# suryatmodulus/livekit-server

Hardware: AMD Instinct MI355X
Metric: forwarded RTP pkts/sec per GPU & node (bit-exact) + % HBM roofline (higher is better)
Workload: dtype u8; 1 GPU; configs[1]: 100 rooms x 10 participants per GPU, VP8 3-layer simulcast + Opus, 18000 DownTracks, 2% loss, 1% reorder, layer switching; batch=1 s of media per step, step=raw datagrams -> Buffer.calc -> forward (lkf_ingest_device + lkf_run), parallelism=room-sharded x1

## Files before the change

### livekit-server_amd/csrc/engine.cpp

```cpp
#include <hip/hip_runtime.h>

#include <algorithm>
#include <chrono>
#include <cmath>
#include <cstdio>
#include <cstdlib>
#include <cstring>
#include <atomic>
#include <map>
#include <mutex>
#include <string>
#include <tuple>
#include <vector>

#include "../../include/lkfwd.h"
#include "ctl_csr.h"
#include "dev_buf.h"
#include "fwd_state.h"
#include "hip_own.h"
#include "kernels.h"

using namespace lkf;

namespace {

struct DevRegistry {
  std::mutex m;
  std::map<uintptr_t, size_t> a;
};
DevRegistry &dreg() {
  static DevRegistry r;
  return r;
}

}

int lkf::dev_alloc(void **p, size_t bytes) {
  *p = nullptr;
  const hipError_t r = hipMalloc(p, bytes);
  if (r == hipSuccess) {
    std::lock_guard<std::mutex> g(dreg().m);
    dreg().a[reinterpret_cast<uintptr_t>(*p)] = bytes;
  }
  return int(r);
}

int lkf::dev_free(void *p) {
  {
    std::lock_guard<std::mutex> g(dreg().m);
    dreg().a.erase(reinterpret_cast<uintptr_t>(p));
  }
  return int(hipFree(p));
}

namespace {

bool dev_range_ok(const void *src, size_t n) {
  const uintptr_t s = reinterpret_cast<uintptr_t>(src);
  std::lock_guard<std::mutex> g(dreg().m);
  auto it = dreg().a.upper_bound(s);
  if (it == dreg().a.begin()) return false;
  --it;
  return s >= it->first && n <= it->second && s - it->first <= it->second - n;
}

constexpr int kStatsWords = 4 + LKF_DROP_NREASONS;
constexpr uint32_t kIdle = 0xffffffffu;

struct Knobs {
  int cuSplit = 0;
// ... 29 lines not shown
    k.debugDD = num("LKF_DEBUG_DD", 0) != 0;
    k.skipBktStore = num("LKF_SKIP_BKT_STORE", 0) != 0;
    k.nackAlone = num("LKF_NACK_ALONE", 0) != 0;
    return k;
  }
};

template <typename Keep>
hipError_t cu_mask_stream(Stream &s, int dev, Keep keep) {
  int ncu = 256;
  (void)hipDeviceGetAttribute(&ncu, hipDeviceAttributeMultiprocessorCount, dev);
  std::vector<uint32_t> m(size_t((ncu + 31) / 32), 0);
  for (int i = 0; i < ncu; i++)
    if (keep(i % 32)) m[size_t(i / 32)] |= 1u << (i % 32);
  return hipExtStreamCreateWithCUMask(s.put(), uint32_t(m.size()), m.data());
}

struct BatchCtx {
  DevBuf<uint32_t> dTBegin, dTEnd, dTRuns, dErr;
  DevBuf<uint64_t> dSlotBase, dPartA, dTot;
  DevBuf<FwdRec> dRecs;
  DevBuf<FwdBase> dFBase;
  DevBuf<FwdBase> dWide;
  DevBuf<uint32_t> dFwdCnt;
  DevBuf<uint64_t> dFwdBytes, dRecBase, dByteBase;
  DevBuf<uint32_t> dGFirst;
  DevBuf<uint32_t> dTwccBase;
  DevBuf<uint32_t> dLayerList, dLayerBefore, dLayerCnt;
  DevBuf<lkf_out> dOut;
  DevBuf<uint8_t> dOutArena;
  int egress = LKF_EGRESS_WIRE;
  DevBuf<lkf_pre> dPre;
  DevBuf<uint32_t> dPreGSum;
  DevBuf<uint64_t> dPreGBase, dPreTot;
  DevBuf<uint64_t> dStats;
  DevBuf<lkf_pkt> dPktsOwn;
  DevBuf<uint8_t> dArenaOwn;
  DevBuf<lkf_raw_pkt> dRawPkts;
  DevBuf<uint64_t> dBktStore;
  DevBuf<lkf_pkt_dd> dDDIn;
  DevBuf<DDPkt> dDDPkt;
  DevBuf<uint8_t> dDDArena;
  DevBuf<uint64_t> dDDUsed;
  DevBuf<uint16_t> dDDSpill;
  DevBuf<DevEvent> dEvents;
  DevBuf<uint32_t> dEvOff;
  DevBuf<uint32_t> dEvLane;
  Event prepped;
  Event pulled;
  Event decided;
  Event sent;
  Event emitted;
  Event ingested;
  bool fromIngest = false;
  bool prepByIngest = false;
  uint32_t prepNT = 0, prepND = 0;
  DevBuf<uint64_t> dITotal;
  bool used = false;
  bool keyed = false;
  DevBuf<uint8_t> dProt;
  bool protectedRun = false;
  DevBuf<RunDesc> dDesc;
  StagePair stage;
  uint32_t stageCap = 0;
  StageGraph gPrep[2], gScan, gCtl;
  void forget_pull_graphs() { gPrep[0].epoch = gPrep[1].epoch = gCtl.epoch = 0; }
};

}

struct lkf_engine {
  int dev = 0;
  Knobs knobs;
  double hp[9] = {};
  CtlCsr csr;
  Stream own;
  Stream d2hS;
  Stream prepS;
  Stream ingS;
  Stream decS;
  Stream emitS;
  Stream sendS;
  Stream sideS;
  std::vector<int32_t> dtTransport;
  DevBuf<uint32_t> dTwccCtrD, dTwccCtrT, dTwccTOff, dTwccTList;
  uint32_t nTwccT = 0;
  bool anyTwcc = false, twccDirty = false;
  Event sideFork, sideDone[2];
  bool sidePending[2] = {false, false};
  Event bktDone[2];
  bool bktPending[2] = {false, false};
  hipStream_t cur = nullptr;
  Event inEv;
  Event bktEv;
  bool bktStorePending = false;
  lkf_cfg cfg{};
  int egress = LKF_EGRESS_WIRE;
  std::string err;

  std::vector<lkf_track_params> tracks;
  std::vector<uint32_t> trackDD;
  std::vector<uint8_t> trackActive;
  std::vector<lkf_downtrack_params> dtp;
  std::vector<uint8_t> active;
  std::vector<uint8_t> seqRM;
  bool schedDirty = true;
// ... 78 lines not shown
  const uint64_t *curNDev = nullptr;
  bool ingestStarted = false;

#ifndef LKF_CTX
#define LKF_CTX 3
#endif
  static constexpr int kCtx = LKF_CTX;
  BatchCtx ctx[kCtx];
  uint64_t nRuns = 0;
  int lastCtx = -1;
  PinnedBuf bounce;

  DevBuf<lkf_nack> dNacks;
  DevBuf<uint32_t> dNackG, dNackValid;
  DevBuf<lkf_rtx> dRtx;
  DevBuf<lkf_raw_pkt> dRtxSrc;
  DevBuf<uint32_t> dRtxLen;
  DevBuf<uint64_t> dRtxOff;
  DevBuf<uint8_t> dRtxIn, dRtxOut;

  DevBuf<TrackerState> dTrk;
  uint32_t nTrk = 0;
  DevBuf<int32_t> dTrkIds;
  DevBuf<lkf_tracker_status> dTrkOut;
  DevBuf<RedEncState> dRedEnc;
  DevBuf<RedDecState> dRedDec;
  struct RedScratch {
    DevBuf<lkf_pkt> in, out;
    DevBuf<uint8_t> inArena, outArena;
    DevBuf<uint32_t> g, cnt;
    DevBuf<int32_t> map;
    DevBuf<uint64_t> off;
  } red;
  DevBuf<lkf_allocation> dLastAlloc;
  DevBuf<lkf_alloc_req> dAllocReq;
  DevBuf<int64_t> dAllocCapacity;
  DevBuf<lkf_allocation> dAllocOut;
  DevBuf<uint8_t> dSrm;
  uint64_t srmStride = 0;
  uint32_t srmCap = 0;
  DevBuf<lkf_pad_req> dPadReq;
  DevBuf<uint64_t> dPadOff;
  DevBuf<uint32_t> dPadCnt;
  DevBuf<lkf_out> dPadOut;
  DevBuf<uint8_t> dPadArena;

  DevBuf<uint16_t> dSns;
  DevBuf<lkf_seq_meta> dSeqOut;
  DevBuf<uint32_t> dSeqN;

  static constexpr int kRing = 256;
  Event ring[kRing][5];
  uint32_t emitGrid = 2048;
  std::vector<lkf_transport_params> transports;
  DevBuf<lkf_transport_params> dTransports;
  DevBuf<SrtpKeys> dSrtpKeys;
  DevBuf<uint32_t> dAesTab;
  DevBuf<SrtpDT> dSrtpDT;
  Event protRing[256][2];
  std::vector<uint8_t> protRun;
  DevBuf<SrtpRx> dSrtpRx, dSrtpRxSpec;
  DevBuf<uint32_t> dRxRange, dRxAuth;
  DevBuf<SrtpRxSpec> dRxSpec;
  DevBuf<lkf_srtp_rx_result> dRxRes;
  DevBuf<uint8_t> dSrtpStage;
  DevBuf<lkf_raw_pkt> dSrtpPktsIn;
  Event rxRing[256][2];
  uint64_t nUnprotects = 0;
  uint32_t lastUnprotectN = 0;
  uint32_t maxStreams = 0;
  DevBuf<DevStream> dStreams;
  DevBuf<StreamHot> dStreamHot;
  DevBuf<uint64_t> dHist;
  DevBuf<uint32_t> dRxGap;
  DevBuf<RangeEntry> dStreamRings;
  DevBuf<uint32_t> dTwcc;
  DevBuf<BucketState> dBkt;
  DevBuf<uint32_t> dBktTag;
  DevBuf<uint64_t> dBktOwner;
  uint32_t bktEpoch = 0;
  DevBuf<uint8_t> dBktRing;
  uint64_t bktSlots = 0;
  DevBuf<int32_t> dBktStream;
  DevBuf<uint16_t> dBktSn;
  DevBuf<uint64_t> dPos, dIPartA, dITotal;
  DevBuf<uint32_t> dITRuns, dIErr;
  struct IngSet {
    DevBuf<IngParsed> parsed;
    DevBuf<lkf_flow> flows;
    DevBuf<uint32_t> fwd, tBegin, tEnd, list, listCnt;
    DevBuf<uint32_t> nackInfo, nackPairOff, nackPairCnt;
    DevBuf<lkf_nack_pair> nackPairs;
    DevBuf<NackIn> nackIn;
  } ing[2];
  int ingPar = 0;
  DevBuf<NackState> dNack;
  uint32_t nackPairCap = 0;
  DevBuf<uint64_t> dNackRecPos, dNackPairPos, dNackTot;
  DevBuf<uint64_t> dNackPartA;
  DevBuf<lkf_rtcp_nack> dNackOut;
  DevBuf<lkf_nack_pair> dNackPairsOut;
  uint32_t lastIngestN = 0;
  const lkf_raw_pkt *ingRaws = nullptr;
  uint32_t nRooms = 0;
  DevBuf<uint32_t> dRoomPartOff, dPartId, dPartMicOff, dMics, dRoomId;
  DevBuf<lkf_speaker> dSpkSlots;
// ... 414 lines not shown
  A(e->dSSGap.alloc(size_t(c.max_downtracks) * kGapWords));
  A(e->dSSRing.alloc(size_t(c.max_downtracks) * kSnInfoSize));
  A(e->dDTs.alloc(c.max_downtracks));
  A(e->dRm.alloc(size_t(c.max_downtracks) * kRangeCap));
  A(e->dVc.alloc(c.max_downtracks));
  A(e->dSeq.alloc(size_t(c.max_downtracks) * c.seq_size));
  e->srmCap = seqrm_cap(c.seq_size);
  e->srmStride = seqrm_stride(e->srmCap);
  A(e->dSrm.alloc(size_t(c.max_downtracks) * e->srmStride));
  A(e->dLastAlloc.alloc(c.max_downtracks));
  A(e->dCum.alloc(kStatsWords));
  A(e->dSticky.alloc(4));
  A(e->dPerm.alloc(c.max_downtracks));
  A(e->dDTOffs.alloc(size_t(c.max_downtracks) * kDTOffsWords));
  const size_t nparts = scan_state_words(c.max_downtracks);
  for (auto &x : e->ctx) {
    A(x.dTBegin.alloc(c.max_tracks));
    A(x.dTEnd.alloc(c.max_tracks));
    A(x.dTRuns.alloc(c.max_tracks));
    A(x.dErr.alloc(4));
    A(x.dSlotBase.alloc(c.max_downtracks));
    A(x.dPartA.alloc(nparts));
    A(hipMemset(x.dPartA, 0, nparts * sizeof(uint64_t)));
    A(x.dTot.alloc(4));
    A(x.dRecs.alloc(c.max_batch_tuples));
    A(x.dFBase.alloc(c.max_downtracks));
    A(x.dWide.alloc(c.max_batch_tuples));
    A(x.dFwdCnt.alloc(c.max_downtracks));
    A(x.dFwdBytes.alloc(c.max_downtracks));
    A(x.dRecBase.alloc(c.max_downtracks));
    A(x.dByteBase.alloc(c.max_downtracks));
    A(x.dGFirst.alloc(c.max_out_pkts / 64 + 2));
    A(x.dTwccBase.alloc(c.max_downtracks));
    A(x.dLayerList.alloc(3 * size_t(c.max_batch_pkts) + 64));
    A(x.dLayerBefore.alloc(3 * size_t(c.max_batch_pkts) + 64));
    A(x.dLayerCnt.alloc(3 * size_t(c.max_tracks)));
    A(x.dOut.alloc(c.max_out_pkts));
    A(x.dOutArena.alloc(c.max_out_bytes + 64));
    A(x.dStats.alloc(size_t(kStatsWords) * (1 + kStatCopies)));
    A(x.dPktsOwn.alloc(c.max_batch_pkts));
    A(x.dArenaOwn.alloc(c.max_batch_arena + 64));
    A(x.dRawPkts.alloc(c.max_batch_pkts));
    A(x.dBktStore.alloc(c.max_batch_pkts));
    A(x.dDesc.alloc(1));
    A(x.dEvents.alloc(4096));
    A(x.dEvLane.alloc(4096));
    A(x.decided.create(false));
    A(x.prepped.create(false));
    A(x.pulled.create(false));
    A(x.emitted.create(false));
    A(x.ingested.create(false));
    A(x.dITotal.alloc(2));
    A(x.sent.create(false));
  }
  for (auto &r : e->ring)
    for (auto &ev : r) A(ev.create(true));
  A(e->scanRead.create(false));
  e->maxStreams = c.max_streams ? c.max_streams : 3 * c.max_tracks;
  A(e->dStreams.alloc(e->maxStreams));
  A(e->dStreamHot.alloc(e->maxStreams));
  A(e->dHist.alloc(size_t(e->maxStreams) * kHistWords));
  A(e->dRxGap.alloc(size_t(e->maxStreams) * kGapWords));
  A(e->dStreamRings.alloc(size_t(e->maxStreams) * kRangeCap));
  for (auto &g : e->ing) {
    A(g.parsed.alloc(c.max_batch_pkts));
    A(g.flows.alloc(c.max_batch_pkts));
    A(g.fwd.alloc(c.max_batch_pkts));
    A(g.tBegin.alloc(c.max_tracks));
    A(g.tEnd.alloc(c.max_tracks));
    A(g.list.alloc(3 * size_t(c.max_batch_pkts) + 64));
    A(g.listCnt.alloc(3 * size_t(c.max_tracks)));
  }
  A(e->dTwcc.alloc(c.max_batch_pkts));
  A(e->dPos.alloc(c.max_batch_pkts));
  const size_t ipart = scan_state_words(c.max_batch_pkts);
  A(e->dIPartA.alloc(ipart));
  A(hipMemset(e->dIPartA, 0, ipart * sizeof(uint64_t)));
  A(e->dITotal.alloc(2));
  A(e->dITRuns.alloc(c.max_tracks));
  A(e->dIErr.alloc(4));
  if (ok) {
    A(hipMemset(e->dSeq, 0, size_t(c.max_downtracks) * c.seq_size * sizeof(SeqMeta)));
    A(hipMemset(e->dRm, 0, size_t(c.max_downtracks) * kRangeCap * sizeof(RangeEntry)));
    A(hipMemset(e->dVc, 0, size_t(c.max_downtracks) * sizeof(VP8Cold)));
    A(hipMemset(e->dSrm, 0, size_t(c.max_downtracks) * e->srmStride));
    A(hipMemset(e->dHot, 0, size_t(c.max_downtracks) * sizeof(DTHot)));
    A(hipMemset(e->dDTs, 0, size_t(c.max_downtracks) * sizeof(DevDT)));
    A(hipMemset(e->dDTCum, 0, size_t(c.max_downtracks) * sizeof(DTCum)));
    A(hipMemset(e->dSeqDDIdx, 0xff, size_t(c.max_downtracks) * sizeof(uint32_t)));
    A(hipMemset(e->dTracks, 0, size_t(c.max_tracks) * sizeof(DevTrack)));
    A(hipMemset(e->dStreamHot, 0, size_t(e->maxStreams) * sizeof(StreamHot)));
    A(hipMemset(e->dStreamRings, 0, size_t(e->maxStreams) * kRangeCap * sizeof(RangeEntry)));
    A(hipMemset(e->dHist, 0, size_t(e->maxStreams) * kHistWords * sizeof(uint64_t)));
    {
      lkf_allocation d = {};
      d.pause_reason = 3;
      d.target_spatial = d.target_temporal = d.request_spatial = d.max_spatial = d.max_temporal = -1;
      std::vector<lkf_allocation> v(c.max_downtracks, d);
      A(hipMemcpy(e->dLastAlloc, v.data(), v.size() * sizeof(lkf_allocation), hipMemcpyHostToDevice));
    }
    A(hipMemset(e->dCum, 0, kStatsWords * sizeof(uint64_t)));
    A(hipMemset(e->dSticky, 0, 4 * sizeof(uint32_t)));
    for (auto &x : e->ctx) {
      A(hipMemset(x.dArenaOwn, 0, c.max_batch_arena + 64));
      A(hipMemset(x.dTot, 0, 4 * sizeof(uint64_t)));
      A(hipMemset(x.dStats, 0, size_t(kStatsWords) * (1 + kStatCopies) * sizeof(uint64_t)));
      A(hipMemset(x.dErr, 0, 4 * sizeof(uint32_t)));
    }
    A(hipDeviceSynchronize());
  }
  if (!ok) {
    lkf_destroy(e);
    return nullptr;
  }
  int cus = 256;
  (void)hipDeviceGetAttribute(&cus, hipDeviceAttributeMultiprocessorCount, hip_device);
  e->emitGrid = uint32_t(cus) * uint32_t(kn.emitWgPerCU);
  return e;
}

void lkf_destroy(lkf_engine *e) {
  if (!e) return;
  if (e->knobs.hostProf && e->hp[5] > 0)
    fprintf(stderr,
            "lkf host ms/run: pre %.4f stage-wait %.4f csr %.4f copies %.4f launches %.4f total %.4f (%d runs)\n",
            e->hp[0] / e->hp[5], e->hp[1] / e->hp[5], e->hp[2] / e->hp[5], e->hp[6] / e->hp[5],
            e->hp[3] / e->hp[5], e->hp[4] / e->hp[5], int(e->hp[5]));
  if (e->knobs.hostProf && e->hp[8] > 0)
    fprintf(stderr, "lkf host ms/ingest: %.4f (%d ingests: the launches of the Buffer.calc chain, no host wait)\n",
            e->hp[7] / e->hp[8], int(e->hp[8]));
  (void)hipSetDevice(e->dev);
  if (e->cur && e->cur != e->own) (void)hipStreamSynchronize(e->cur);
  if (e->own) (void)hipStreamSynchronize(e->own);
  if (e->ingS) (void)hipStreamSynchronize(e->ingS);
  if (e->prepS) (void)hipStreamSynchronize(e->prepS);
  if (e->decS) (void)hipStreamSynchronize(e->decS);
  if (e->emitS) (void)hipStreamSynchronize(e->emitS);
  if (e->sendS) (void)hipStreamSynchronize(e->sendS);
  if (e->sideS) (void)hipStreamSynchronize(e->sideS);
  if (e->d2hS) (void)hipStreamSynchronize(e->d2hS);
  (void)hipDeviceSynchronize();
  delete e;
}

int32_t lkf_add_track(lkf_engine *e, const lkf_track_params *p) {
  if (!e || !p) return LKF_EINVAL;
  if (e->tracks.size() >= e->cfg.max_tracks) return LKF_ENOSPC;
  int32_t h = int32_t(e->tracks.size());
  e->tracks.push_back(*p);
  uint32_t ddIdx = 0xffffffffu;
  if (track_has_dd(*p)) ddIdx = e->nDDTracks++;
  e->trackDD.push_back(ddIdx);
  e->trackActive.push_back(1);
  e->trkSR.emplace_back();
  std::memcpy(e->trkSR.back().offs, p->layer_offsets, 9 * sizeof(uint32_t));
  e->pendTracks.push_back(to_dev_track(*p, ddIdx));
  e->schedDirty = true;
  return h;
}

static bool at_key_valid(int32_t kind, int64_t key) {
  if (kind == LKF_AT_PKT) return key >= 0 && key <= int64_t(0xffffffffu);
  if (kind == LKF_AT_DATAGRAM) return key >= 0;
  return kind == LKF_AT_ARRIVAL_NS;
}

int lkf_set_layer_offsets_key(lkf_engine *e, int32_t track, const uint32_t offsets[9], int32_t kind, int64_t key) {
  if (!e || !offsets || track < 0 || track >= int32_t(e->tracks.size())) return LKF_EINVAL;
  if (!at_key_valid(kind, key)) return LKF_EINVAL;
  lkf_engine::TrackOp op;
  op.track = uint32_t(track);
  op.at = kind == LKF_AT_PKT ? uint32_t(key) : 0u;
  op.kind = kind;
  op.key = key;
  std::memcpy(op.offs, offsets, sizeof(op.offs));
  std::memcpy(e->trkSR[size_t(track)].offs, offsets, sizeof(op.offs));
  e->trkOps.push_back(op);
  if (kind != LKF_AT_PKT) e->keyedPending = true;
  return LKF_OK;
}
// ... 726 lines not shown
    q.list = e->dSeqDDList;
    q.n = e->nSeqDD;
    q.hot = e->dHot;
    q.seq = e->dSeq;
    q.seqSize = e->cfg.seq_size;
    q.srm = e->dSrm;
    q.srmStride = e->srmStride;
    q.srmCap = e->srmCap;
    q.ddIdx = e->dSeqDDIdx;
    q.seqDD = e->dSeqDD;
    q.recs = x.dRecs;
    q.fbase = x.dFBase;
    q.wide = x.dWide;
    q.slotBase = x.dSlotBase;
    q.fwdCnt = x.dFwdCnt;
    q.pkts = e->curPkts;
    q.ddArena = x.dDDArena;
    HIPCHK(launch_seq_dd(s, q), "sequencer dd");
  }
  return LKF_OK;
}

static EmitArgs emit_args(const lkf_engine *e, const BatchCtx &x, const RunCtx &r) {
  EmitArgs m{};
  m.perm = e->dPerm;
  m.recBase = x.dRecBase;
  m.byteBase = x.dByteBase;
  m.gFirst = x.dGFirst;
  m.slotBase = x.dSlotBase;
  m.totals = x.dTot + 2;
  m.recs = x.dRecs;
  m.fbase = x.dFBase;
  m.wide = x.dWide;
  m.pkts = e->curPkts;
  m.arena = e->curArena;
  m.dts = e->dDTs;
  m.ndts = r.nd;
  m.out = x.dOut;
  m.outArena = x.dOutArena;
  m.outCap = e->cfg.max_out_pkts;
  m.outByteCap = e->cfg.max_out_bytes;
  m.err = x.dErr;
  m.ddArena = e->ddAlloc ? x.dDDArena.get() : nullptr;
  m.maxDts = e->cfg.max_downtracks;
  m.npkts = e->curN;
  m.tupleCap = e->cfg.max_batch_tuples;
  m.arenaLen = e->curArenaLen;
  m.ddCap = x.dDDArena.cap();
  m.twccBase = e->anyTwcc ? x.dTwccBase.get() : nullptr;
  m.gCap = e->cfg.max_out_pkts / 64 + 2;
  return m;
}

static uint32_t emit_grid(const lkf_engine *e) {
  return e->knobs.emitPersistent ? e->emitGrid : uint32_t(((e->cfg.max_out_pkts + 63) / 64 + 7) / 8 * 8);
}

static uint32_t emit_lds_pad(const lkf_engine *e, const RunCtx &r) {
  const bool lowFanout = uint64_t(r.nd) < uint64_t(e->knobs.emitCapFanout) * std::max<uint32_t>(1, r.nt);
  return r.ingestFed && lowFanout ? e->knobs.emitLdsPad : 0;
}

static int enqueue_emit(lkf_engine *e, BatchCtx &x, const RunCtx &r) {
  hipStream_t es = e->emitS;
  HIPCHK(hipStreamWaitEvent(es, x.decided, 0), "wait decided");
  HIPCHK(hipEventRecord(r.rg[3], es), "event");
  const EmitArgs m = emit_args(e, x, r);
  const uint32_t grid = emit_grid(e);
  x.egress = e->egress;
  if (x.egress == LKF_EGRESS_PREFIX) {
    EmitPrefixLaunch q;
    q.pre = x.dPre;
    q.gSum = x.dPreGSum;
    q.gBase = x.dPreGBase;
    q.total = x.dPreTot;
    if (r.nd)
      HIPCHK(launch_emit_prefix(es, m, grid, q), "emit prefix");
    else
      HIPCHK(hipMemsetAsync(x.dPreTot, 0, sizeof(uint64_t), es), "emit prefix");
  } else if (r.nd) {
    HIPCHK(launch_emit(es, m, grid, emit_lds_pad(e, r)), "emit");
  }
  HIPCHK(hipEventRecord(r.rg[4], es), "event");
  HIPCHK(launch_accumulate(es, x.dStats, x.dTot, e->dCum, x.dErr, e->dSticky), "accumulate");
  if (e->bktStorePending) {
    HIPCHK(hipEventRecord(x.sent, e->sendS), "event");
    HIPCHK(hipStreamWaitEvent(es, x.sent, 0), "wait bucket store");
  }
  e->bktStorePending = false;
  HIPCHK(hipEventRecord(x.emitted, es), "event");
  return LKF_OK;
}

static void finish_run(lkf_engine *e, BatchCtx &x, const RunCtx &r) {
  if (e->knobs.hostProf && e->nRuns >= 3) {
    e->hp[0] += ms_between(r.tp0, r.tp1);
    e->hp[1] += ms_between(r.tp1, r.tp2);
    e->hp[2] += ms_between(r.tp2, r.tp25);
    e->hp[6] += ms_between(r.tp25, r.tp3);
    e->hp[3] += ms_since(r.tp3);
    e->hp[4] += ms_since(r.tp0);
    e->hp[5] += 1;
  }
  x.used = true;
  x.protectedRun = false;
  if (!e->protRun.empty()) e->protRun[e->nRuns % 256] = 0;
  e->lastCtx = r.ci;
  e->nRuns++;
  e->haveBatch = false;
  e->curNDev = nullptr;
  e->curDD = nullptr;
}

int lkf_run(lkf_engine *e, void *stream) {
  if (!e) return LKF_EINVAL;
  HIPCHK(hipSetDevice(e->dev), "hipSetDevice");
  if (int rc = flush_topology(e)) return rc;
  if (e->schedDirty) {
    if (int rc = rebuild_sched(e)) return rc;
  }
  if (e->twccDirty) {
    if (int rc = rebuild_twcc(e)) return rc;
  }
  RunCtx r{};
  r.ci = int(e->nRuns % lkf_engine::kCtx);
  BatchCtx &x = e->ctx[r.ci];
  if (!e->haveBatch) {
    e->curPkts = x.dPktsOwn;
    e->curArena = x.dArenaOwn;
    e->curOwned = e->curDDOwned = true;
    e->curN = 0;
    e->curNDev = nullptr;
    e->curArenaLen = 0;
    e->curFromIngest = false;
  }
  r.tp0 = clk::now();
  hipStream_t us = stream ? reinterpret_cast<hipStream_t>(stream) : e->own;
  e->cur = us;
  r.nt = uint32_t(e->tracks.size());
  r.nd = uint32_t(e->dtp.size());
  r.nl = uint32_t(e->sched.size());
  r.rg = e->ring[e->nRuns % lkf_engine::kRing];
  expand_track_ops(e, r);
  r.keyed = e->keyedPending;
  e->keyedPending = false;
  if (r.keyed) {
    if (int rc = refuse_mixed_kinds(e, r)) return rc;
  }
  for (const auto &op : e->trkOps)
    std::memcpy(e->tracks[op.track].layer_offsets, op.offs, sizeof(op.offs));
  e->trkOps.clear();
  if (int rc = wait_inputs(e, x, r, us)) return rc;
  if (int rc = stage_ctl(e, x, r)) return rc;
  if (int rc = enqueue_prep(e, x, r)) return rc;
  if (int rc = enqueue_decide(e, x, r)) return rc;
// ... 2636 lines not shown
```

### livekit-server_amd/csrc/forward_kernels.hip

```cpp
#include <hip/hip_runtime.h>

#include "../../include/lkfwd.h"
#ifndef LKF_SVC_STATS
#define LKF_SVC_STATS 0
#endif
#if LKF_SVC_STATS
__device__ unsigned long long g_svc[64 * 48];
#define SVC_ADD(k, v) atomicAdd(&g_svc[(blockIdx.x & 63) * 48 + (k)], (unsigned long long)(v))
#endif
#include "dd_device.h"
#include "fwd_state.h"
#include "kernels.h"
#include "sender_device.h"

namespace lkf {

using u8 = uint8_t;
using u16 = uint16_t;
using u32 = uint32_t;
using u64 = uint64_t;
using i32 = int32_t;
using i64 = int64_t;

constexpr u64 HALF64 = 1ull << 63;
// ... 4083 lines not shown
    u32 lo = b, hi = e;
    while (lo < hi) {
      const u32 mid = lo + ((hi - lo) >> 1);
      if (R.pkts[mid].arrival_ns < k.key)
        lo = mid + 1;
      else
        hi = mid;
    }
    return lo < e ? lo : kEnd;
  }
  return at;
}
__global__ void __launch_bounds__(256) k_ev_resolve(EvResolve R, DevEvent *__restrict__ evs,
                                                    const u32 *__restrict__ laneOf, u32 nev) {
  const u32 i = blockIdx.x * blockDim.x + threadIdx.x;
  if (i >= nev) return;
  const u32 at = ev_resolve_one(R, R.keys[i], evs[i].at);
#if LKF_CHECKED
  if (i && laneOf[i - 1] == laneOf[i]) {
    const DevKey kp = R.keys[i - 1];
    const u32 prev = ev_resolve_one(R, kp, kp.kind == LKF_AT_PKT ? evs[i - 1].at : 0u);
    CHK(prev <= at, CK_EV_ORDER, i, prev);
  }
#endif
  if (R.keys[i].kind != LKF_AT_PKT) evs[i].at = at;
}

hipError_t launch_ev_resolve(hipStream_t s, const DevKey *keys, DevEvent *evs, const u32 *laneOf, u32 nev,
                             const lkf_pkt *pkts, const u32 *tBegin, const u32 *tEnd, u32 ntracks, const u64 *pos,
                             u32 nRaw) {
  if (!nev) return hipSuccess;
  EvResolve R;
  R.keys = keys;
  R.pkts = pkts;
  R.tBegin = tBegin;
  R.tEnd = tEnd;
  R.pos = pos;
  R.ntracks = ntracks;
  R.nRaw = nRaw;
  hipLaunchKernelGGL(k_ev_resolve, dim3((nev + 255) / 256), dim3(256), 0, s, R, evs, laneOf, nev);
  return hipGetLastError();
}

hipError_t launch_ev_offsets(hipStream_t s, const u32 *laneOf, const RunDesc *desc, u32 nl, u32 *off) {
  hipLaunchKernelGGL(k_ev_offsets, dim3((nl + 1 + 255) / 256), dim3(256), 0, s, laneOf, desc, nl, off);
  return hipGetLastError();
}

hipError_t launch_stats_reduce(hipStream_t s, u64 *stats) {
  hipLaunchKernelGGL(k_stats_reduce, dim3(1), dim3(256), 0, s, stats);
  return hipGetLastError();
}

__global__ void k_accumulate(const u64 *stats, const u64 *tot, u64 *cum, const u32 *err, u32 *sticky) {
  const int i = threadIdx.x;
  if (i < 4 + LKF_DROP_NREASONS) cum[i] += (i == 3) ? tot[3] : stats[i];
  if (i == 0 && err[0]) sticky[0] |= err[0] & 0xffu;
}

__global__ void k_err_fold(const u32 *err, u32 *sticky, u32 shift) {
  if (threadIdx.x == 0 && err[0]) sticky[0] |= (err[0] & 0xffu) << shift;
}

hipError_t launch_err_fold(hipStream_t s, const u32 *err, u32 *sticky, u32 shift) {
  hipLaunchKernelGGL(k_err_fold, dim3(1), dim3(64), 0, s, err, sticky, shift);
  return hipGetLastError();
}

__device__ void dd_tracker_observe(DDTrkState &T, const DDStruct &S, const DDPkt &o, u32 ddFlags, u32 pktSize,
                                   u32 payload) {
  if ((T.flags & (DT_PAUSED | DT_STOPPED)) || payload == 0) return;
  if ((o.flags & DP_ACTIVE) && (ddFlags & LKF_DD_ACTIVE_UPDATED)) {
    i32 ms = 0, mt = 0;
    for (u32 k = 0; k < S.numDT; k++)
      if (o.activeMask & (1u << S.dtTarget[k])) {
        ms = max(ms, i32(S.dtS[k]));
        mt = max(mt, i32(S.dtT[k]));
      }
    ms = min(ms, 2);
    mt = min(mt, 3);
    const i32 old = T.maxS;
    T.maxS = ms;
    T.maxT = mt;
    if (old == -1) T.flags |= DT_WORKER;
    const i32 lo = old > ms ? ms + 1 : old + 1, hi = old > ms ? old : ms;
    for (i32 l = lo; l <= hi && old != ms; l++) {
      T.notif[l]++;
      T.lastNotified[l] = old > ms ? 0 : 1;
    }
  }
  for (u32 k = 0; k < S.numDT; k++) {
    const u32 tg = S.dtTarget[k];
    if (o.ndti <= tg || ((o.dtis >> (2 * tg)) & 3) == 0) continue;
    T.bytes[S.dtS[k]][S.dtT[k]] += pktSize;
  }
}

__global__ void __launch_bounds__(64) k_dd_decode(const RunDesc *__restrict__ desc, const u32 *__restrict__ tBegin,
                                                  const u32 *__restrict__ tEnd, const DevTrack *__restrict__ tracks,
                                                  u32 ntracks, DDStruct *structs, DDTrack *ddTracks,
                                                  DDPkt *__restrict__ out, u32 *err,
                                                  const u32 *__restrict__ trackDDTrk, DDTrkState *ddTrk, u16 *spill,
                                                  u32 *spillUsed, u32 spillCap) {
  const lkf_pkt *__restrict__ pkts = reinterpret_cast<const lkf_pkt *>(desc->pkts);
  const lkf_pkt_dd *__restrict__ dds = reinterpret_cast<const lkf_pkt_dd *>(desc->dd);
  const u8 *__restrict__ arena = reinterpret_cast<const u8 *>(desc->arena);
  const u32 t = blockIdx.x, lane = threadIdx.x;
  if (t >= ntracks) return;
  const u32 ddIdx = tracks[t].ddIdx;
  if (ddIdx == 0xffffffffu) return;
// ... 297 lines not shown

hipError_t launch_emit(hipStream_t s, const EmitArgs &a, u32 grid, u32 ldsPad) {
  if (a.ddArena)
    hipLaunchKernelGGL(k_emit<PRE_MAX_DD>, dim3(grid), dim3(EMIT_T), 0, s, a);
  else
    hipLaunchKernelGGL(k_emit<PRE_MAX>, dim3(grid), dim3(EMIT_T), ldsPad, s, a);
  return hipGetLastError();
}

hipError_t launch_emit_prefix(hipStream_t s, const EmitArgs &a, u32 grid, const EmitPrefixLaunch &x) {
  EmitPreArgs P;
  P.e = a;
  P.e.out = nullptr;
  P.pre = x.pre;
  P.gSum = x.gSum;
  P.gBase = x.gBase;
  P.preTotal = x.total;
  if (a.ddArena)
    hipLaunchKernelGGL(k_emit_prelen<PRE_MAX_DD>, dim3(grid), dim3(EMIT_T), 0, s, P);
  else
    hipLaunchKernelGGL(k_emit_prelen<PRE_MAX>, dim3(grid), dim3(EMIT_T), 0, s, P);
  hipLaunchKernelGGL(k_emit_prescan, dim3(1), dim3(PRESCAN_T), 0, s, P);
  if (a.ddArena)
    hipLaunchKernelGGL(k_emit_prefix<PRE_MAX_DD>, dim3(grid), dim3(EMIT_T), 0, s, P);
  else
    hipLaunchKernelGGL(k_emit_prefix<PRE_MAX>, dim3(grid), dim3(EMIT_T), 0, s, P);
  return hipGetLastError();
}

__global__ void k_h2d(const u8 *__restrict__ stage, RunDesc *__restrict__ dDesc, DevEvent *__restrict__ dEv,
                      u32 *__restrict__ dLane) {
  const RunDesc *h = reinterpret_cast<const RunDesc *>(stage);
  const u32 nev = h->nev, cap = h->evCap;
  const u64 nA = u64(nev) * (sizeof(DevEvent) / 4), nB = nev;
  const u32 *sA = reinterpret_cast<const u32 *>(stage + stage_ev_off(cap));
  const u32 *sB = reinterpret_cast<const u32 *>(stage + stage_lane_off(cap));
  u32 *dA = reinterpret_cast<u32 *>(dEv);
  const u64 stride = u64(gridDim.x) * blockDim.x;
  const u64 t = u64(blockIdx.x) * blockDim.x + threadIdx.x;
  if (t < sizeof(RunDesc) / 4) reinterpret_cast<u32 *>(dDesc)[t] = reinterpret_cast<const u32 *>(h)[t];
  for (u64 i = t; i < nA + nB; i += stride) {
    if (i < nA)
      dA[i] = sA[i];
    else
      dLane[i - nA] = sB[i - nA];
  }
}

hipError_t launch_h2d(hipStream_t s, const uint8_t *stage, RunDesc *dDesc, DevEvent *dEv, uint32_t *dLane) {
  hipLaunchKernelGGL(k_h2d, dim3(256), dim3(256), 0, s, stage, dDesc, dEv, dLane);
  return hipGetLastError();
}

hipError_t launch_accumulate(hipStream_t s, const u64 *stats, const u64 *tot, u64 *cum, const u32 *err, u32 *sticky) {
  hipLaunchKernelGGL(k_accumulate, dim3(1), dim3(64), 0, s, stats, tot, cum, err, sticky);
  return hipGetLastError();
}

hipError_t launch_seq_lookup(hipStream_t s, DTHot *hot, SeqMeta *seq, u32 seqSize, u8 *srm, u64 srmStride, u32 srmCap,
                             u32 d, const u16 *sns, u32 n, i64 nowMs, lkf_seq_meta *out, u32 *nOut) {
  hipLaunchKernelGGL(k_seq_lookup, dim3(1), dim3(64), 0, s, hot, seq, seqSize, srm, srmStride, srmCap, d, sns, n, nowMs,
                     out, nOut);
  return hipGetLastError();
}

}
```

### livekit-server_amd/csrc/hip_own.h

```cpp
#pragma once
#include <hip/hip_runtime.h>

#include <cstdlib>

namespace lkf {

template <typename H>
struct Owned {
  H h = nullptr;
  Owned() = default;
  Owned(const Owned &) = delete;
  Owned &operator=(const Owned &) = delete;
  operator H() const { return h; }
  H get() const { return h; }
};

struct Event : Owned<hipEvent_t> {
  ~Event() { reset(); }
  hipError_t create(bool timing) {
    reset();
    return timing ? hipEventCreate(&h) : hipEventCreateWithFlags(&h, hipEventDisableTiming);
  }
  void reset() {
    if (h) (void)hipEventDestroy(h);
// ... 27 lines not shown
    h = nullptr;
    return r;
  }
  void reset() { (void)destroy(); }
};

struct StageGraph {
  GraphExec exec;
  uint64_t epoch = 0;
};

struct StagePair {
  uint8_t *host = nullptr, *dev = nullptr;
  StagePair() = default;
  StagePair(const StagePair &) = delete;
  StagePair &operator=(const StagePair &) = delete;
  ~StagePair() { reset(); }
  hipError_t alloc(size_t n) {
    reset();
    const size_t bytes = (n + 4095) & ~size_t(4095);
    void *p = std::aligned_alloc(4096, bytes);
    if (!p) return hipErrorOutOfMemory;
    hipError_t r = hipHostRegister(p, bytes, hipHostRegisterMapped);
    void *d = nullptr;
    if (r == hipSuccess && (r = hipHostGetDevicePointer(&d, p, 0)) != hipSuccess) (void)hipHostUnregister(p);
    if (r != hipSuccess) {
      std::free(p);
      return r;
    }
    host = static_cast<uint8_t *>(p);
    dev = static_cast<uint8_t *>(d);
    return hipSuccess;
  }
  void reset() {
    if (host) {
      (void)hipHostUnregister(host);
      std::free(host);
    }
    host = dev = nullptr;
  }
};

struct PinnedBuf {
  uint8_t *p = nullptr;
  PinnedBuf() = default;
  PinnedBuf(const PinnedBuf &) = delete;
  PinnedBuf &operator=(const PinnedBuf &) = delete;
  ~PinnedBuf() {
    if (p) (void)hipHostFree(p);
  }
  hipError_t alloc(size_t bytes) { return hipHostMalloc(reinterpret_cast<void **>(&p), bytes, hipHostMallocDefault); }
};

}
```

### livekit-server_amd/csrc/kernels.h

```cpp
#pragma once
#include <hip/hip_runtime.h>

#include "../../include/lkfwd.h"
#include "fwd_state.h"
#include "srtp_rx_device.h"

namespace lkf {

struct DecideArgs {
  const uint32_t *sched;
  const uint32_t *waveTrack;
  uint32_t nlanes;
  DTHot *hot;
  const DevDT *dts;
  const DevTrack *tracks;
  RangeEntry *rm;
  VP8Cold *vc;
  SeqMeta *seq;
  uint32_t seqSize;
  uint8_t *srm;
  uint64_t srmStride;
  uint32_t srmCap;
  const lkf_pkt *pkts;
  const uint32_t *tBegin, *tEnd;
// ... 156 lines not shown
                               uint64_t *partA, uint64_t *partB, uint64_t *recPos, uint64_t *pairPos, uint64_t *totals,
                               lkf_rtcp_nack *outRecs, lkf_nack_pair *outPairs);

struct SpeakersLaunch {
  uint32_t nrooms;
  const uint32_t *roomPartOff, *partId, *partMicOff, *mics, *roomId;
  const DevStream *streams;
  StreamHot *hot;
  int64_t nowNs;
  lkf_speaker *slots;
  uint32_t *counts;
};

hipError_t launch_ingest(hipStream_t s, const IngestLaunch &a, hipStream_t side, hipEvent_t sideFork,
                         hipEvent_t sideDone, bool *sideUsed);
hipError_t launch_speakers(hipStream_t s, const SpeakersLaunch &a);
struct RoomPackLaunch {
  uint32_t rows, k, s;
  const int32_t *rowEng;
  const lkf_speaker *slots;
  const uint32_t *counts;
  const uint32_t *slotOff, *slotDts;
  const int64_t *slotSub;
  const DTCum *cum;
  int32_t *spk;
  int64_t *bwe;
};
hipError_t launch_room_pack(hipStream_t spkStream, hipStream_t bweStream, const RoomPackLaunch &a);
hipError_t launch_decide(hipStream_t s, DecideArgs a, uint32_t ddLanes);
hipError_t launch_layer_index(hipStream_t s, const RunDesc *desc, const uint32_t *tBegin, const uint32_t *tEnd,
                              uint32_t ntracks, uint32_t stride, uint32_t *list, uint32_t *before, uint32_t *cnt,
                              uint64_t *zero2 = nullptr);
hipError_t launch_emit(hipStream_t s, const EmitArgs &a, uint32_t grid, uint32_t ldsPad);
struct EmitPrefixLaunch {
  lkf_pre *pre;
  uint32_t *gSum;
  uint64_t *gBase;
  uint64_t *total;
};
hipError_t launch_emit_prefix(hipStream_t s, const EmitArgs &a, uint32_t grid, const EmitPrefixLaunch &x);
hipError_t launch_dd_decode(hipStream_t s, const RunDesc *desc, const uint32_t *tBegin, const uint32_t *tEnd,
                            const DevTrack *tracks, uint32_t ntracks, DDStruct *structs, DDTrack *ddTracks, DDPkt *out,
                            uint32_t *err, const uint32_t *trackDDTrk, DDTrkState *ddTrk, uint16_t *spill,
                            uint32_t *spillUsed, uint32_t spillCap);
hipError_t launch_dd_tracker_tick(hipStream_t s, DDTrkState *st, const int32_t *ids, uint32_t n, int64_t elapsedNs,
                                  lkf_dd_tracker_status *out);
hipError_t launch_h2d(hipStream_t s, const uint8_t *stage, RunDesc *dDesc, DevEvent *dEv, uint32_t *dLane);
hipError_t launch_stats_reduce(hipStream_t s, uint64_t *stats);
hipError_t launch_ev_offsets(hipStream_t s, const uint32_t *laneOf, const RunDesc *desc, uint32_t nl, uint32_t *off);
hipError_t launch_ev_resolve(hipStream_t s, const DevKey *keys, DevEvent *evs, const uint32_t *laneOf, uint32_t nev,
                             const lkf_pkt *pkts, const uint32_t *tBegin, const uint32_t *tEnd, uint32_t ntracks,
                             const uint64_t *pos, uint32_t nRaw);
hipError_t launch_accumulate(hipStream_t s, const uint64_t *stats, const uint64_t *tot, uint64_t *cum,
                             const uint32_t *err, uint32_t *sticky);
hipError_t launch_err_fold(hipStream_t s, const uint32_t *err, uint32_t *sticky, uint32_t shift);
hipError_t launch_rtx_lookup(hipStream_t s, const DTHot *hot, SeqMeta *seq, uint32_t seqSize, uint8_t *srm,
                             uint64_t srmStride, uint32_t srmCap, const lkf_nack *nacks,
                             const uint32_t *gStart, uint32_t ngroups, int64_t nowMs, lkf_rtx *out, uint32_t *valid);
hipError_t launch_rtx_emit(hipStream_t s, bool write, uint32_t n, const lkf_rtx *rtx, const lkf_raw_pkt *src,
                           const uint8_t *arena, const DevDT *dts, const DevTrack *tracks, uint32_t *lens,
                           const uint64_t *offs, uint8_t *out, const uint8_t *dd);
struct SrtpKeys {
  uint32_t rk[44];
  uint32_t ih[5];
  uint32_t oh[5];
  uint32_t salt[4];
  uint32_t profile;
  uint32_t pad[5];
};
static_assert(sizeof(SrtpKeys) == 256, "SrtpKeys is 256 B");
struct SrtpDT {
  uint32_t tp1;
  uint32_t init;
  uint64_t rocBase;
};
struct SrtpProtectArgs {
  const uint32_t *tab;
  const uint64_t *totals;
  const lkf_out *out;
  const uint8_t *arena;
  uint8_t *prot;
  const DevDT *dts;
  SrtpDT *sd;
  const SrtpKeys *keys;
  uint64_t cap;
  uint32_t absVal;
};
hipError_t launch_aes_tables(hipStream_t s, uint32_t *tab);
hipError_t launch_srtp_keys(hipStream_t s, const lkf_transport_params *in, uint32_t first, uint32_t n,
                            const uint32_t *tab, SrtpKeys *keys);
hipError_t launch_srtp_protect(hipStream_t s, const SrtpProtectArgs &a, uint32_t ndts, const uint32_t *perm,
                               const uint64_t *recBase, const uint32_t *fwdCnt);

struct SrtpRxSpec {
  uint64_t v;
  uint32_t st;
  uint32_t h;
};
struct SrtpRxArgs {
  const uint32_t *tab;
  const lkf_raw_pkt *pkts;
  uint32_t n;
  uint32_t nstreams;
  const uint8_t *srtp;
  uint64_t srtpLen;
  lkf_raw_pkt *pktsOut;
  uint8_t *plain;
// ... 198 lines not shown
```

Before: 1.520 billion forwarded RTP pkts/s.

## Size emit grid from recent output counts via mapped host slot

The non-persistent emit kernel used to launch a grid sized for the worst-case output capacity (max_out_pkts/64 workgroups). Now the accumulate kernel writes each run's output-packet count plus a sequence number into a pinned, mapped host slot. The host then sizes the next emit grid from the largest recent count, with a 1/16 margin, a residency-based floor, and the capacity as ceiling. This removes idle workgroups that scan empty slots. The risk is correctness if output grows past the margin, unless the emit kernel grid-strides over the remainder.

```diff
diff --git a/livekit-server_amd/csrc/emit_grid.h b/livekit-server_amd/csrc/emit_grid.h
--- /dev/null
+++ b/livekit-server_amd/csrc/emit_grid.h
@@ -0,0 +1,54 @@
+#pragma once
+#include <cstdint>
+
+namespace lkf {
+
+constexpr uint32_t kEmitGroup = 64;
+constexpr uint32_t kEmitGridAlign = 8;
+constexpr uint32_t kEmitWgPerCU = 24;
+constexpr uint32_t kEmitWgPerCUCapped = 12;
+constexpr uint64_t kEmitGridMax = 0x7ffffff8ull;
+
+struct EmitSlot {
+  static uint64_t pack(uint32_t seq, uint64_t count) {
+    return (uint64_t(seq) << 32) | (count > 0xffffffffull ? 0xffffffffull : count);
+  }
+  static uint32_t seq(uint64_t v) { return uint32_t(v >> 32); }
+  static uint32_t count(uint64_t v) { return uint32_t(v); }
+};
+
+inline uint64_t emit_round_up(uint64_t v, uint64_t a) { return (v + a - 1) / a * a; }
+
+inline uint64_t emit_groups_grid(uint64_t records) {
+  const uint64_t g = emit_round_up(records / kEmitGroup + (records % kEmitGroup ? 1 : 0), kEmitGridAlign);
+  return g ? g : kEmitGridAlign;
+}
+
+inline uint32_t emit_capacity_grid(uint64_t maxOutPkts) {
+  const uint64_t g = emit_groups_grid(maxOutPkts);
+  return uint32_t(g > kEmitGridMax ? kEmitGridMax : g);
+}
+
+inline uint32_t emit_floor_grid(uint32_t capGrid, uint32_t cus, bool capped) {
+  const uint64_t resident = emit_round_up(uint64_t(cus ? cus : 1) * (capped ? kEmitWgPerCUCapped : kEmitWgPerCU),
+                                          kEmitGridAlign);
+  uint64_t quarter = emit_round_up(uint64_t(capGrid) / 4, kEmitGridAlign);
+  if (quarter < kEmitGridAlign) quarter = kEmitGridAlign;
+  uint64_t f = resident < quarter ? resident : quarter;
+  if (f > capGrid) f = capGrid;
+  return uint32_t(f);
+}
+
+inline uint32_t emit_grid_size(const uint32_t *counts, int n, uint32_t capGrid, uint32_t cus, bool capped) {
+  if (n <= 0) return capGrid;
+  uint64_t most = 0;
+  for (int i = 0; i < n; i++) most = counts[i] > most ? counts[i] : most;
+  const uint64_t groups = most / kEmitGroup + (most % kEmitGroup ? 1 : 0);
+  uint64_t g = most ? emit_round_up(groups + groups / 16, kEmitGridAlign) + kEmitGridAlign : 0;
+  const uint32_t fl = emit_floor_grid(capGrid, cus, capped);
+  if (g < fl) g = fl;
+  if (g > capGrid) g = capGrid;
+  return uint32_t(g);
+}
+
+}
diff --git a/livekit-server_amd/csrc/emit_grid_unit.cpp b/livekit-server_amd/csrc/emit_grid_unit.cpp
--- /dev/null
+++ b/livekit-server_amd/csrc/emit_grid_unit.cpp
@@ -0,0 +1,185 @@
+#include <cstdio>
+#include <cstdlib>
+#include <cstring>
+#include <string>
+#include <vector>
+
+#include "emit_grid.h"
+
+using namespace lkf;
+
+static int g_fail = 0;
+#define CHECK(c)                                                  \
+  do {                                                            \
+    if (!(c)) {                                                   \
+      std::printf("  %s:%d: CHECK(%s)\n", __FILE__, __LINE__, #c); \
+      g_fail++;                                                   \
+    }                                                             \
+  } while (0)
+
+static const uint64_t kCaps[] = {1,       63,        64,         65,          2048,        3500,
+                                 65536,   1u << 20,  3862528,    (1ull << 31) + 5,
+                                 0xffffffffull - 64, 0xffffffffull - 1, 0xffffffffull};
+static const uint32_t kCus[] = {1, 8, 104, 256, 304};
+
+static uint32_t grid1(uint32_t count, uint32_t capGrid, uint32_t cus, bool capped) {
+  return emit_grid_size(&count, 1, capGrid, cus, capped);
+}
+
+static void no_history_is_capacity() {
+  for (uint64_t cap : kCaps)
+    for (uint32_t cus : kCus)
+      for (int capped = 0; capped < 2; capped++) {
+        const uint32_t cg = emit_capacity_grid(cap);
+        CHECK(emit_grid_size(nullptr, 0, cg, cus, capped) == cg);
+        const uint32_t some[2] = {5, 7};
+        CHECK(emit_grid_size(some, 0, cg, cus, capped) == cg);
+        CHECK(emit_grid_size(some, -1, cg, cus, capped) == cg);
+      }
+  CHECK(emit_capacity_grid(3862528) == 60352);
+  CHECK(emit_capacity_grid(64) == 8 && emit_capacity_grid(65) == 8 && emit_capacity_grid(513) == 16);
+}
+
+static std::vector<uint32_t> sweep_counts(uint64_t cap) {
+  std::vector<uint32_t> v = {0, 1, 63, 64, 65, 511, 512, 513, 1790, 100000, 1080000};
+  for (uint64_t c : {cap / 16, cap / 4, cap / 2, cap - (cap ? 1 : 0), cap, cap + 1, cap * 2})
+    v.push_back(uint32_t(c > 0xffffffffull ? 0xffffffffull : c));
+  v.push_back(0xffffffffu);
+  return v;
+}
+
+static void multiple_of_8_within_bounds() {
+  for (uint64_t cap : kCaps)
+    for (uint32_t cus : kCus)
+      for (int capped = 0; capped < 2; capped++) {
+        const uint32_t cg = emit_capacity_grid(cap), fl = emit_floor_grid(cg, cus, capped);
+        CHECK(cg % 8 == 0 && cg >= 8);
+        CHECK(fl % 8 == 0 && fl >= 8 && fl <= cg);
+        for (uint32_t c : sweep_counts(cap)) {
+          const uint32_t g = grid1(c, cg, cus, capped);
+          CHECK(g % 8 == 0);
+          CHECK(g >= fl && g <= cg);
+          const uint32_t h3[3] = {c / 2, c, c / 3}, h3b[3] = {c, 0, c / 2};
+          CHECK(emit_grid_size(h3, 3, cg, cus, capped) == g);
+          CHECK(emit_grid_size(h3b, 3, cg, cus, capped) == g);
+        }
+      }
+}
+
+static void monotone_in_largest_count() {
+  for (uint64_t cap : kCaps)
+    for (uint32_t cus : kCus)
+      for (int capped = 0; capped < 2; capped++) {
+        const uint32_t cg = emit_capacity_grid(cap);
+        std::vector<uint32_t> cs = sweep_counts(cap);
+        for (uint32_t a : cs)
+          for (uint32_t b : cs)
+            if (a <= b) CHECK(grid1(a, cg, cus, capped) <= grid1(b, cg, cus, capped));
+        uint32_t prev = 0;
+        for (uint32_t c = 0; c < 4096; c++) {
+          const uint32_t g = grid1(c, cg, cus, capped);
+          CHECK(g >= prev);
+          prev = g;
+        }
+      }
+}
+
+static void zero_count_is_floor() {
+  for (uint64_t cap : kCaps)
+    for (uint32_t cus : kCus)
+      for (int capped = 0; capped < 2; capped++) {
+        const uint32_t cg = emit_capacity_grid(cap);
+        CHECK(grid1(0, cg, cus, capped) == emit_floor_grid(cg, cus, capped));
+        const uint32_t z[3] = {0, 0, 0};
+        CHECK(emit_grid_size(z, 3, cg, cus, capped) == emit_floor_grid(cg, cus, capped));
+      }
+  CHECK(emit_floor_grid(60352, 256, true) == 3072);
+  CHECK(emit_floor_grid(60352, 256, false) == 6144);
+  CHECK(emit_floor_grid(32, 256, false) == 8);
+  CHECK(emit_floor_grid(8, 256, false) == 8);
+}
+
+static void count_at_capacity_is_capacity() {
+  for (uint64_t cap : kCaps)
+    for (uint32_t cus : kCus)
+      for (int capped = 0; capped < 2; capped++) {
+        const uint32_t cg = emit_capacity_grid(cap);
+        CHECK(grid1(uint32_t(cap), cg, cus, capped) == cg);
+        CHECK(grid1(0xffffffffu, cg, cus, capped) == cg);
+      }
+}
+
+static void margin_covers_growth() {
+  for (uint32_t c : {1080000u, 128000u, 20000u}) {
+    const uint32_t cg = emit_capacity_grid(uint64_t(c) * 4);
+    const uint32_t g = grid1(c, cg, 256, true);
+    const uint64_t grown = (uint64_t(c) * 105 / 100 + 63) / 64;
+    CHECK(g >= grown || g == emit_floor_grid(cg, 256, true));
+    CHECK(g <= (c + 63) / 64 * 17 / 16 + 24 || g == emit_floor_grid(cg, 256, true));
+  }
+}
+
+static void no_overflow_near_2_32() {
+  CHECK(emit_capacity_grid(0xffffffffull) == 67108864u);
+  CHECK(emit_capacity_grid(0xffffffffull - 62) == 67108864u);
+  CHECK(emit_capacity_grid(0xffffffffull - 63) == 67108864u - 0);
+  CHECK(emit_capacity_grid(1ull << 32) == 67108864u);
+  CHECK(emit_capacity_grid(~0ull) == 0x7ffffff8u);
+  const uint32_t cg = emit_capacity_grid(0xffffffffull);
+  CHECK(grid1(0xffffffffu, cg, 256, false) == cg);
+  CHECK(grid1(0xffffffffu - 64, cg, 256, false) == cg);
+  const uint32_t g = grid1(0xf0000000u, cg, 256, false);
+  CHECK(g == 62914560u + 62914560u / 16 + 8);
+  const uint32_t h = grid1(0x80000000u, cg, 256, false);
+  CHECK(h == (0x80000000u / 64) / 16 * 17 + 8);
+  CHECK(emit_floor_grid(0x7ffffff8u, 0xffffffffu, false) <= 0x7ffffff8u);
+  CHECK(EmitSlot::count(EmitSlot::pack(7, 1ull << 40)) == 0xffffffffu);
+  CHECK(EmitSlot::seq(EmitSlot::pack(7, 1ull << 40)) == 7);
+  CHECK(EmitSlot::count(EmitSlot::pack(0xffffffffu, 123)) == 123 && EmitSlot::seq(EmitSlot::pack(0xffffffffu, 123)) == 0xffffffffu);
+}
+
+struct Case {
+  const char *name;
+  void (*fn)();
+};
+static const Case kCases[] = {
+    {"grid_no_history_is_capacity", no_history_is_capacity},
+    {"grid_multiple_of_8_within_bounds", multiple_of_8_within_bounds},
+    {"grid_monotone_in_largest_count", monotone_in_largest_count},
+    {"grid_zero_count_is_floor", zero_count_is_floor},
+    {"grid_count_at_capacity_is_capacity", count_at_capacity_is_capacity},
+    {"grid_margin_covers_growth", margin_covers_growth},
+    {"grid_no_overflow_near_2_32", no_overflow_near_2_32},
+};
+
+int main(int argc, char **argv) {
+  if (argc > 1 && !std::strcmp(argv[1], "--list")) {
+    for (const Case &c : kCases) std::printf("%s\n", c.name);
+    return 0;
+  }
+  if (argc > 1 && !std::strcmp(argv[1], "--grid")) {
+    if (argc < 5) return 2;
+    const uint64_t cap = std::strtoull(argv[2], nullptr, 10);
+    const uint32_t cus = uint32_t(std::strtoul(argv[3], nullptr, 10));
+    const bool capped = std::atoi(argv[4]) != 0;
+    std::vector<uint32_t> counts;
+    for (int i = 5; i < argc; i++) counts.push_back(uint32_t(std::strtoul(argv[i], nullptr, 10)));
+    const uint32_t cg = emit_capacity_grid(cap);
+    std::printf("%u %u %u\n", emit_grid_size(counts.data(), int(counts.size()), cg, cus, capped),
+                emit_floor_grid(cg, cus, capped), cg);
+    return 0;
+  }
+  int ran = 0;
+  for (const Case &c : kCases) {
+    if (argc > 1 && std::strcmp(argv[1], c.name)) continue;
+    const int before = g_fail;
+    c.fn();
+    ran++;
+    std::printf("%s %s\n", g_fail == before ? "PASS" : "FAIL", c.name);
+  }
+  if (!ran) {
+    std::printf("no such case\n");
+    return 2;
+  }
+  return g_fail ? 1 : 0;
+}
diff --git a/livekit-server_amd/csrc/engine.cpp b/livekit-server_amd/csrc/engine.cpp
--- a/livekit-server_amd/csrc/engine.cpp
+++ b/livekit-server_amd/csrc/engine.cpp
@@ -16,6 +16,7 @@
 #include "../../include/lkfwd.h"
 #include "ctl_csr.h"
 #include "dev_buf.h"
+#include "emit_grid.h"
 #include "fwd_state.h"
 #include "hip_own.h"
 #include "kernels.h"
@@ -151,6 +152,8 @@
   Event sent;
   Event emitted;
   Event ingested;
+  HostSlot emitSlot;
+  uint64_t slotRun[2] = {0, 0};
   bool fromIngest = false;
   bool prepByIngest = false;
   uint32_t prepNT = 0, prepND = 0;
@@ -335,6 +338,11 @@
   static constexpr int kRing = 256;
   Event ring[kRing][5];
   uint32_t emitGrid = 2048;
+  uint32_t cus = 256;
+  uint64_t emitHistFrom = 0;
+  uint32_t emitHistND = 0;
+  uint32_t lastEmitGrid = 0;
+  double emitGridSum = 0;
   std::vector<lkf_transport_params> transports;
   DevBuf<lkf_transport_params> dTransports;
   DevBuf<SrtpKeys> dSrtpKeys;
@@ -855,6 +863,7 @@
     A(x.ingested.create(false));
     A(x.dITotal.alloc(2));
     A(x.sent.create(false));
+    A(x.emitSlot.alloc(1));
   }
   for (auto &r : e->ring)
     for (auto &ev : r) A(ev.create(true));
@@ -919,6 +928,7 @@
   int cus = 256;
   (void)hipDeviceGetAttribute(&cus, hipDeviceAttributeMultiprocessorCount, hip_device);
   e->emitGrid = uint32_t(cus) * uint32_t(kn.emitWgPerCU);
+  e->cus = uint32_t(cus);
   return e;
 }
 
@@ -929,6 +939,9 @@
             "lkf host ms/run: pre %.4f stage-wait %.4f csr %.4f copies %.4f launches %.4f total %.4f (%d runs)\n",
             e->hp[0] / e->hp[5], e->hp[1] / e->hp[5], e->hp[2] / e->hp[5], e->hp[6] / e->hp[5],
             e->hp[3] / e->hp[5], e->hp[4] / e->hp[5], int(e->hp[5]));
+  if (e->knobs.hostProf && e->hp[5] > 0)
+    fprintf(stderr, "lkf emit grid: %.0f workgroups per launch on average, %u the last (capacity %u)\n",
+            e->emitGridSum / e->hp[5], e->lastEmitGrid, lkf::emit_capacity_grid(e->cfg.max_out_pkts));
   if (e->knobs.hostProf && e->hp[8] > 0)
     fprintf(stderr, "lkf host ms/ingest: %.4f (%d ingests: the launches of the Buffer.calc chain, no host wait)\n",
             e->hp[7] / e->hp[8], int(e->hp[8]));
@@ -1761,13 +1774,37 @@
   return m;
 }
 
-static uint32_t emit_grid(const lkf_engine *e) {
-  return e->knobs.emitPersistent ? e->emitGrid : uint32_t(((e->cfg.max_out_pkts + 63) / 64 + 7) / 8 * 8);
+static bool emit_capped(const lkf_engine *e, const RunCtx &r) {
+  const bool lowFanout = uint64_t(r.nd) < uint64_t(e->knobs.emitCapFanout) * std::max<uint32_t>(1, r.nt);
+  return r.ingestFed && lowFanout;
+}
+
+#ifndef LKF_EMIT_CAPGRID
+#define LKF_EMIT_CAPGRID 0
+#endif
+static uint32_t emit_grid(lkf_engine *e, const RunCtx &r) {
+  if (e->knobs.emitPersistent) return e->emitGrid;
+  const uint32_t capGrid = lkf::emit_capacity_grid(e->cfg.max_out_pkts);
+  if (r.nd > e->emitHistND) e->emitHistFrom = e->nRuns + 1;
+  e->emitHistND = r.nd;
+  if (LKF_EMIT_CAPGRID) return capGrid;
+  uint32_t counts[lkf_engine::kCtx];
+  int n = 0;
+  for (const BatchCtx &x : e->ctx) {
+    const uint64_t v = __atomic_load_n(x.emitSlot.host, __ATOMIC_RELAXED);
+    const uint32_t seq = lkf::EmitSlot::seq(v);
+    if (!seq) continue;
+    for (const uint64_t run : x.slotRun)
+      if (run && uint32_t(run) == seq && run >= e->emitHistFrom) {
+        counts[n++] = lkf::EmitSlot::count(v);
+        break;
+      }
+  }
+  return lkf::emit_grid_size(counts, n, capGrid, e->cus, emit_capped(e, r));
 }
 
 static uint32_t emit_lds_pad(const lkf_engine *e, const RunCtx &r) {
-  const bool lowFanout = uint64_t(r.nd) < uint64_t(e->knobs.emitCapFanout) * std::max<uint32_t>(1, r.nt);
-  return r.ingestFed && lowFanout ? e->knobs.emitLdsPad : 0;
+  return emit_capped(e, r) ? e->knobs.emitLdsPad : 0;
 }
 
 static int enqueue_emit(lkf_engine *e, BatchCtx &x, const RunCtx &r) {
@@ -1775,7 +1812,8 @@
   HIPCHK(hipStreamWaitEvent(es, x.decided, 0), "wait decided");
   HIPCHK(hipEventRecord(r.rg[3], es), "event");
   const EmitArgs m = emit_args(e, x, r);
-  const uint32_t grid = emit_grid(e);
+  const uint32_t grid = emit_grid(e, r);
+  e->lastEmitGrid = grid;
   x.egress = e->egress;
   if (x.egress == LKF_EGRESS_PREFIX) {
     EmitPrefixLaunch q;
@@ -1791,7 +1829,10 @@
     HIPCHK(launch_emit(es, m, grid, emit_lds_pad(e, r)), "emit");
   }
   HIPCHK(hipEventRecord(r.rg[4], es), "event");
-  HIPCHK(launch_accumulate(es, x.dStats, x.dTot, e->dCum, x.dErr, e->dSticky), "accumulate");
+  x.slotRun[1] = x.slotRun[0];
+  x.slotRun[0] = e->nRuns + 1;
+  HIPCHK(launch_accumulate(es, x.dStats, x.dTot, e->dCum, x.dErr, e->dSticky, x.emitSlot.dev, uint32_t(e->nRuns + 1)),
+         "accumulate");
   if (e->bktStorePending) {
     HIPCHK(hipEventRecord(x.sent, e->sendS), "event");
     HIPCHK(hipStreamWaitEvent(es, x.sent, 0), "wait bucket store");
@@ -1810,6 +1851,7 @@
     e->hp[3] += ms_since(r.tp3);
     e->hp[4] += ms_since(r.tp0);
     e->hp[5] += 1;
+    e->emitGridSum += e->lastEmitGrid;
   }
   x.used = true;
   x.protectedRun = false;
diff --git a/livekit-server_amd/csrc/forward_kernels.hip b/livekit-server_amd/csrc/forward_kernels.hip
--- a/livekit-server_amd/csrc/forward_kernels.hip
+++ b/livekit-server_amd/csrc/forward_kernels.hip
@@ -4159,10 +4159,12 @@
   return hipGetLastError();
 }
 
-__global__ void k_accumulate(const u64 *stats, const u64 *tot, u64 *cum, const u32 *err, u32 *sticky) {
+__global__ void k_accumulate(const u64 *stats, const u64 *tot, u64 *cum, const u32 *err, u32 *sticky, u64 *slot,
+                             u32 seq) {
   const int i = threadIdx.x;
   if (i < 4 + LKF_DROP_NREASONS) cum[i] += (i == 3) ? tot[3] : stats[i];
   if (i == 0 && err[0]) sticky[0] |= err[0] & 0xffu;
+  if (i == 0) *slot = (u64(seq) << 32) | (tot[2] > 0xffffffffull ? 0xffffffffull : tot[2]);
 }
 
 __global__ void k_err_fold(const u32 *err, u32 *sticky, u32 shift) {
@@ -4566,8 +4568,9 @@
   return hipGetLastError();
 }
 
-hipError_t launch_accumulate(hipStream_t s, const u64 *stats, const u64 *tot, u64 *cum, const u32 *err, u32 *sticky) {
-  hipLaunchKernelGGL(k_accumulate, dim3(1), dim3(64), 0, s, stats, tot, cum, err, sticky);
+hipError_t launch_accumulate(hipStream_t s, const u64 *stats, const u64 *tot, u64 *cum, const u32 *err, u32 *sticky,
+                             u64 *slot, u32 seq) {
+  hipLaunchKernelGGL(k_accumulate, dim3(1), dim3(64), 0, s, stats, tot, cum, err, sticky, slot, seq);
   return hipGetLastError();
 }
 
diff --git a/livekit-server_amd/csrc/hip_own.h b/livekit-server_amd/csrc/hip_own.h
--- a/livekit-server_amd/csrc/hip_own.h
+++ b/livekit-server_amd/csrc/hip_own.h
@@ -103,4 +103,27 @@
   hipError_t alloc(size_t bytes) { return hipHostMalloc(reinterpret_cast<void **>(&p), bytes, hipHostMallocDefault); }
 };
 
+struct HostSlot {
+  uint64_t *host = nullptr, *dev = nullptr;
+  HostSlot() = default;
+  HostSlot(const HostSlot &) = delete;
+  HostSlot &operator=(const HostSlot &) = delete;
+  ~HostSlot() {
+    if (host) (void)hipHostFree(host);
+  }
+  hipError_t alloc(size_t words) {
+    void *p = nullptr, *d = nullptr;
+    hipError_t r = hipHostMalloc(&p, words * sizeof(uint64_t), hipHostMallocMapped | hipHostMallocCoherent);
+    if (r != hipSuccess) return r;
+    if ((r = hipHostGetDevicePointer(&d, p, 0)) != hipSuccess) {
+      (void)hipHostFree(p);
+      return r;
+    }
+    host = static_cast<uint64_t *>(p);
+    dev = static_cast<uint64_t *>(d);
+    for (size_t i = 0; i < words; i++) host[i] = 0;
+    return hipSuccess;
+  }
+};
+
 }
diff --git a/livekit-server_amd/csrc/kernels.h b/livekit-server_amd/csrc/kernels.h
--- a/livekit-server_amd/csrc/kernels.h
+++ b/livekit-server_amd/csrc/kernels.h
@@ -232,7 +232,7 @@
                              const lkf_pkt *pkts, const uint32_t *tBegin, const uint32_t *tEnd, uint32_t ntracks,
                              const uint64_t *pos, uint32_t nRaw);
 hipError_t launch_accumulate(hipStream_t s, const uint64_t *stats, const uint64_t *tot, uint64_t *cum,
-                             const uint32_t *err, uint32_t *sticky);
+                             const uint32_t *err, uint32_t *sticky, uint64_t *slot, uint32_t seq);
 hipError_t launch_err_fold(hipStream_t s, const uint32_t *err, uint32_t *sticky, uint32_t shift);
 hipError_t launch_rtx_lookup(hipStream_t s, const DTHot *hot, SeqMeta *seq, uint32_t seqSize, uint8_t *srm,
                              uint64_t srmStride, uint32_t srmCap, const lkf_nack *nacks,
```

Measured after the change: 1.499 billion forwarded RTP pkts/s. 0.986x the previous value.
